# Farama-Foundation/Procgen2

Measured on AMD Instinct MI355X. Metric: env-steps/sec at 65536 envs, 64x64x3 obs, higher is better.
Workload: dtype u8/f32; 1 GPU; coinrun, 65536 envs per GPU, uniform random actions 0..14 from a device counter hash, next-step auto-reset, seeds 1+global env index; game=coinrun, distribution_mode=default, envs_per_gpu=65536, obs=64x64x3 uint8, parallelism=env-shard x1, no collective

## Files before the change

procgen2_amd/csrc/coinrun.hip:

```cpp
#include "../../include/procgen2_vec.h"
#include "pg_engine.h"
#include "pg_frame.h"
#include "pg_geom.h"
#include "pg_order.h"
#include "pg_prefetch.h"
#include "pg_prepass.h"
#include "pg_render.h"
#include "pg_rng.h"
#include "pg_tiles.h"

namespace pg {
namespace PG_VARIANT_NS {
namespace coinrun {

constexpr int W = 64, H = 64;
constexpr int kMaxEnt = 36;
constexpr int kSparks = 10;
constexpr int kSparkRow = 12;

enum Tile : uint8_t { kEmpty = 0, kWallTop, kWallMid, kLavaTop, kLavaMid, kCrate };
enum Solid { kPass = 0, kFull, kOneWay };
enum Kind { kSaw = 0, kMob = 1, kCoin = 2 };

enum Tex {
// ... 836 lines not shown
#pragma unroll
    for (int ss = 0; ss < 4; ss++) {
        bx[ss] = SC(s, SC_AX + ss, env) + -0.5f;
        by[ss] = SC(s, SC_AY + ss, env) + -1.0f;
    }
    int hazard = 0;
    if (cand0 | cand1) {
        SCI(s, SC_CAND, env) = 0;
        SCI(s, SC_CAND + 1, env) = 0;
    }
    if (bits & kBitsFar) {
        const int n_ent = SI(s, I_NENT, env);
        for (int e = 0; e < n_ent; e++) {
            float hb[6];
            entity_step<false>(s, env, e, src, 4, hb);
            hazard |= hazard_hits(hb, bx, by);
        }
    } else {
        unsigned long long cand = cand0 | (static_cast<unsigned long long>(cand1) << 32);
        while (cand) {
            const int e = __builtin_ctzll(cand);
            cand &= cand - 1;
            const float4 x = s.hazx[size_t(e) * s.n + env];
            const float2 y = s.hazy[size_t(e) * s.n + env];
            const float hb[6] = {x.x, x.y, x.z, x.w, y.x, y.y};
            hazard |= hazard_hits(hb, bx, by);
        }
    }
    const int lava = (bits >> 8) & 15, coin = (bits >> 12) & 15;
    const int ending = hazard | lava | coin;
    const int last = ending ? __builtin_ctz(ending) : 3;
    SCI(s, SC_REDO, env) = last < 3 ? last + 1 : 0;
    const bool alive = !(((hazard | lava) >> last) & 1);
    const bool got_coin = ((coin >> last) & 1) != 0;
    const float ax = SC(s, SC_AX + last, env), ay = SC(s, SC_AY + last, env);
    SF(s, F_AX, env) = ax;
    SF(s, F_AY, env) = ay;
    SF(s, F_AVX, env) = SC(s, SC_AVX + last, env);
    SF(s, F_AVY, env) = SC(s, SC_AVY + last, env);
    SF(s, F_APHASE, env) = SC(s, SC_PHASE + last, env);
    SF(s, F_CAMX, env) = ax * kUnitPx;
    SF(s, F_CAMY, env) = (ay - 0.5f) * kUnitPx;
    SI(s, I_FLAGS, env) = kFlagListed | (((bits >> last) & 1) ? kFlagGround : 0) |
                          (((bits >> (4 + last)) & 1) ? kFlagForward : 0) | (src ? 0 : kFlagBuf);
    const bool terminated = !alive || got_coin;
    io.reward[env] = got_coin * 10.0f;
    io.done[env] = terminated ? 1 : 0;
    io.pending[env] = terminated ? reset_due_mark(step_index + 1u) : 0;
}

constexpr int kRenderWaves = 2;
#ifndef PG_COINRUN_QUARTERS
#define PG_COINRUN_QUARTERS false
#endif
constexpr bool kQuarters = PG_COINRUN_QUARTERS;

#ifndef PG_COINRUN_RENDER_WAVES
#define PG_COINRUN_RENDER_WAVES 5
#endif
constexpr int kGrid = 16;

PG_D int tile_tex(int tile, int crate, int ground_theme) {
    return tile == kWallMid   ? kTexMid + ground_theme
           : tile == kWallTop ? kTexTop + ground_theme
           : tile == kLavaMid ? kTexLava
           : tile == kLavaTop ? kTexLavaTop
                              : kTexCrate + crate;
}
PG_D int kind_tex(int k, int ground_theme) { return tile_tex(k < 4 ? k + 1 : kCrate, (k - 4) & 3, ground_theme); }
PG_D DrawCall spark_draw(float life, float x, float y, const int4& d) {
    if (!(life > 0.0f)) return kNoDraw;
    const float lr = (5.0f - life) / 5.0f;
    const float alpha = 0.5f * (1.0f - lr);
    const float scale = 0.45f * (0.4f * lr + 0.6f);
    const float oy = -lr * 0.17f;
    return DrawCall{true, false, false, kTexSpark, x * kUnitPx - 0.5f * d.y * scale, (y + oy) * kUnitPx - 0.5f * d.z * scale,
                    scale * kUnitPx / d.y, alpha, 0.0f};
}
PG_D int sprite_tex(int tex0, int dyn) { return (dyn & kDynTexSet) ? tex0 + ((dyn & kDynFrame) ? 1 : 0) : 0; }
PG_D DrawCall sprite_draw(int dyn, float x, float y, int tex, const int4& d) {
    if (!(dyn & kDynTexSet)) return kNoDraw;
    const float scale = 1.0f * 1.0f;
    return DrawCall{true, (dyn & kDynFlip) != 0, false, tex, (x + -0.5f) * kUnitPx, (y + -0.5f) * kUnitPx, scale * kUnitPx / d.y, 1.0f, 0.0f};
}
PG_D int agent_tex(int sflags, float avx, float aphase, int alien) {
    const bool ground = (sflags & kFlagGround) != 0;
    if (fabsf(avx) < 0.01f && ground) return kTexStand + alien;
    if (!ground) return kTexJump + alien;
    return (aphase > 0.5f ? kTexWalk2 : kTexWalk1) + alien;
}
PG_D DrawCall agent_draw(int sflags, float ax, float ay, int tex, const int4& d) {
    const float px = ax - 0.5f, py = ay - 2.0f;
    return DrawCall{true, (sflags & kFlagForward) == 0, false, tex, px * kUnitPx, py * kUnitPx, kUnitPx / d.y, 1.0f, 0.0f};
}

PG_D void render_full(const State& s, const AtlasView& atlas, const StepIO& io, int flags, int env, uint32_t* fb,
                      ComposeLds<kGrid>& L) {
    const int lane = threadIdx.x & 63, half = __builtin_amdgcn_readfirstlane(threadIdx.x >> 6);
    constexpr int halves = kRenderWaves;
    uint32_t* const slots = fb + kFbWords - kBlitWords * 64;
    static_assert(sizeof(ComposeTmp<kGrid>) + sizeof(ComposeHand) + kBlitWords * 64 * 4 <= kFbWords * 4, "room behind the set-up tables");

    const Camera cam{SF(s, F_CAMX, env), SF(s, F_CAMY, env), 64.0f, 64.0f, 0.3f * 64.0f / 64.0f};
    const int themes = SI(s, I_THEMES, env);
    const int sflags = SI(s, I_FLAGS, env);
    const int buf = (sflags & kFlagBuf) ? 1 : 0;
    const int backdrop = PG_ABL(flags, 16) ? 9 : (themes & 0xff);
    const int alien = (themes >> 8) & 0xff, ground_theme = (themes >> 16) & 0xff;
    const int n_ent = SI(s, I_NENT, env);
    const int n_mob = SI(s, I_NMOB, env);
    const uint8_t* tiles = s.tiles + size_t(env) * (W * H);
    const DescRegs descs = DescRegs::load(atlas, lane);
    Blit mine;
    PG_MARK("a_state");

    {
        const int redo = SCI(s, SC_REDO, env);
        __syncthreads();
        if (redo) {
            if (half == 0 && lane < n_ent) {
                float hb[6];
                entity_step(s, env, lane, 1 - buf, redo, hb);
            }
            if (threadIdx.x == 0) SCI(s, SC_REDO, env) = 0;
            __threadfence();
            __syncthreads();
        }
    }

    const int n_parts = n_mob * kSparks;
    const int n_sprites = (sflags & kFlagListed) ? n_ent : 0;
    const bool one_pass = n_parts + n_sprites + 1 <= 64;
    const int first_sprite = one_pass ? n_parts : 0;
    const bool is_part = one_pass && lane < n_parts;
    const bool is_sprite = lane >= first_sprite && lane < first_sprite + n_sprites;
    const bool is_agent = lane == first_sprite + n_sprites;
    int spr_e = 0, spr_dyn = 0, spr_tex = 0;
    float spr_x = 0.0f, spr_y = 0.0f, part_life = 0.0f, part_x = 0.0f, part_y = 0.0f;
    if (half != 1) {
    } else if (is_sprite) {
        spr_e = EB(s, EB_DRAW_ORDER, lane - first_sprite, env);
        spr_dyn = DB(s, buf, spr_e, env);
        spr_tex = EB(s, EB_TEX, spr_e, env);
        spr_x = DF(s, buf, DF_X, spr_e, env);
        spr_y = EY(s, spr_e, env);
    } else if (is_part) {
        const int m = lane / kSparks, k = lane - m * kSparks;
        const int e = EB(s, EB_SPARK_ORDER, m, env);
        part_life = SP(s, buf, 2, e, k, env);
        part_x = SP(s, buf, 0, e, k, env);
        part_y = SP(s, buf, 1, e, k, env);
    }
    PG_MARK("b_inputs");

    const BgDraw bg_draw = backdrop_draw(descs.uniform(kTexBackdrop + backdrop), SF(s, F_BGSHIFT, env));
    const int4& bg_d = bg_draw.desc;

    const TileWindow win = tile_window(cam);
    const int x0 = win.x0, y0 = win.y0;
    const int cols = win.x1 - x0 + 1, rows = win.y1 - y0 + 1, cells = cols * rows;
    const int4 tile_desc = descs.uniform(kTexMid);

    if (half == 1 && !PG_ABL(flags, 2)) {
        {
            bool has = false;
            int want_tex = 0;
            if (is_part)
                want_tex = kTexSpark;
            else if (is_sprite)
                want_tex = sprite_tex(spr_tex, spr_dyn);
            else if (is_agent)
                want_tex = agent_tex(sflags, SF(s, F_AVX, env), SF(s, F_APHASE, env), alien);
            const int4 d = descs.at(want_tex);
            DrawCall c = kNoDraw;
            if (is_part)
                c = spark_draw(part_life, part_x, part_y, d);
            else if (is_sprite)
                c = sprite_draw(spr_dyn, spr_x, spr_y, want_tex, d);
            else if (is_agent)
                c = agent_draw(sflags, SF(s, F_AX, env), SF(s, F_AY, env), want_tex, d);
            if (c.go) has = resolve_draw(cam, d.y, d.z, d.x, c.wx, c.wy, c.scale, c.alpha, c.flip_h, false, mine);
            blit_share(slots, lane, mine, has);
        }
    }
    PG_MARK("c_resolve");
    BgAxis bga{};
    bool composed = false, sprites_ready = false;
    ReplayState<4> sprite_pass;
    if (!(flags & 1) && !PG_ABL(flags, 4) && cols <= kGrid && rows <= kGrid) {
        compose_spans(fb, L, cam, x0, y0, cols, rows, tile_desc.y, tile_desc.z, kUnitPx / tile_desc.y, lane, 0, half, halves,
                      0, 0, &bg_draw, &bga);
    PG_MARK("d_spans");
        const int4 kind_d = descs.at(kind_tex(lane & 7, ground_theme));
        const int kind_base = kind_d.x;
        uint32_t soft_rows = (threadIdx.x == 0 && bg_d.w != 0) ? 0x80000000u : 0u;
        const uint32_t hard_rows = (threadIdx.x == 0 && (bg_d.w & 2)) ? 0x80000000u : 0u;
#pragma unroll
        for (int k = 0; k < kGrid * kGrid / 64; k++) {
            if (half != 0) break;
            const int cell = k * 64 + lane;
            const int r = cell / kGrid, c = cell % kGrid;
            const int x = x0 + c, ty = H - 1 - (y0 + r);
            int raw = kWallMid;
            if (x >= 0 && ty >= 0 && x < W && ty < H) raw = tiles[ty + x * H];
            const int t = raw & 7;
            const int slot = t < kCrate ? t - 1 : 4 + (raw >> 4);
            const int off = __shfl(kind_base, slot < 0 ? 0 : slot);
            const int soft = __shfl(kind_d.w, slot < 0 ? 0 : slot);
            L.base[cell] = (t == kEmpty) ? static_cast<int32_t>(kNoTexel) : off * 4;
            if (t != kEmpty && soft != 0 && r < rows && c < cols) soft_rows |= 1u << r;
        }
        if (soft_rows) atomicOr(&L.soft_rows[half], static_cast<int32_t>(soft_rows));
        if (hard_rows) atomicOr(&L.hard_rows[half], static_cast<int32_t>(hard_rows));
        __syncthreads();
        PG_MARK("e_cells");
        sprites_ready = !PG_ABL(flags, 2);
        if (sprites_ready) {
            const bool has = blit_take(slots, lane, mine);
            sprite_pass = replay_begin(atlas, mine, __ballot(has), lane, half * (kObsH / halves), (half + 1) * (kObsH / halves));
        }
        PG_MARK("f_begin");
        composed = compose_rows(fb, L, atlas, bga, cols, rows, tile_desc.y, lane, flags, half, halves);
        PG_MARK("k_composed");
    }
    if (PG_ABL(flags, 4)) composed = true;
    bool taken = false;
    if (!composed) {
        if (!sprites_ready) {
            __syncthreads();
            taken = blit_take(slots, lane, mine);
            __syncthreads();
        }
        Blit tile;
        wave_clear(fb, lane, half, halves);
        const bool has_bg = resolve_draw(cam, bg_d.y, bg_d.z, bg_d.x, bg_draw.px, bg_draw.py, bg_draw.scale, 1.0f, false, false, tile);
        wave_replay(fb, atlas, tile, has_bg ? 1ull : 0ull, lane, half, halves);
        for (int base = 0; base < cells; base += 64) {
            const int cell = base + lane;
            bool has = false;
            if (cell < cells) {
                const int row = cell / cols;
                const int x = x0 + (cell - row * cols), y = y0 + row;
                const int ty = H - 1 - y;
                int t = kWallMid, crate = 0;
                if (x >= 0 && ty >= 0 && x < W && ty < H) {
                    const int raw = tiles[ty + x * H];
                    t = raw & 7;
                    crate = raw >> 4;
                }
                if (t != kEmpty) {
                    const int4 d = atlas.desc[tile_tex(t, crate, ground_theme)];
                    has = resolve_draw(cam, d.y, d.z, d.x, x * kUnitPx, y * kUnitPx, kUnitPx / d.y, 1.0f, false, false,
                                       tile);
                }
            }
            wave_replay(fb, atlas, tile, __ballot(has), lane, half, halves);
        }
    }

    if (!PG_ABL(flags, 2)) {
        const int4 spark_d = descs.uniform(kTexSpark);
        if (!one_pass) {
            Blit spark;
            for (int base = 0; base < n_parts; base += 64) {
                bool has = false;
                if (base + lane < n_parts) {
                    const int idx = base + lane, m = idx / kSparks, k = idx - m * kSparks;
                    const int e = EB(s, EB_SPARK_ORDER, m, env);
                    const DrawCall c = spark_draw(SP(s, buf, 2, e, k, env), SP(s, buf, 0, e, k, env), SP(s, buf, 1, e, k, env), spark_d);
                    has = c.go && resolve_draw(cam, spark_d.y, spark_d.z, spark_d.x, c.wx, c.wy, c.scale, c.alpha, false, false, spark);
                }
                wave_replay_rows(fb, atlas, spark, __ballot(has), lane, half * (kObsH / halves), (half + 1) * (kObsH / halves));
            }
        }
        if (!sprites_ready)
            sprite_pass = replay_begin(atlas, mine, __ballot(taken), lane, half * (kObsH / halves), (half + 1) * (kObsH / halves));
        PG_MARK("m_fallback_and_rounds");
        replay_finish(fb, atlas, mine, sprite_pass, lane, half * (kObsH / halves), (half + 1) * (kObsH / halves));
        PG_MARK("n_sprites");
    }
    if (!PG_ABL(flags, 8))
        wave_store_rows(fb, io.obs + size_t(env) * kObsBytes, lane, half * (kObsH / halves), (half + 1) * (kObsH / halves));
    PG_MARK("o_store");
}

constexpr int kPrepEnvs = 8, kPrepThreads = 256;
constexpr int kSlotTop = 0, kSlotMid = 1, kSlotLavaTop = 2, kSlotLava = 3, kSlotCrate = 4;

struct PrepEnv {
    int32_t sflags, buf, n_ent, n_mob, n_sprites, alien;
    float avx, aphase, ax, ay;
};
struct SetupLds {
    PrepLds<kGrid, kPrepEnvs, kMaxSpan> P;
    PrepEnv env[kPrepEnvs];
    int4 desc[kTexCount];
    uint8_t order[kPrepEnvs][2][kMaxEnt + 4];
    int32_t kind_soft[kPrepEnvs];
    uint32_t row_valid[kPrepEnvs][kGrid / 4];
    int32_t counts[kPrepEnvs];
    PrepDrawQueue queue[kPrepThreads / 64];
};

__global__ void __launch_bounds__(kPrepThreads) setup_kernel(State s, AtlasView atlas, const uint8_t* mask, int flags) {
    __shared__ SetupLds S;
    PrepLds<kGrid, kPrepEnvs, kMaxSpan>& P = S.P;
    const int tid = threadIdx.x, lane = tid & 63, wave = __builtin_amdgcn_readfirstlane(tid >> 6);
    const int env0 = prep_block(blockIdx.x, gridDim.x) * kPrepEnvs;
    const PrepOut& out = s.prep;

    for (int q = tid; q < kPrepEnvs * 2 * 64; q += kPrepThreads) (&P.cover[0][0][0])[q] = 0u;
    if (tid < kTexCount) S.desc[tid] = atlas.desc[tid];
    static_assert(kTexCount <= kPrepThreads, "one descriptor per thread");
    for (int q = tid; q < kPrepEnvs * 2 * kMaxEnt; q += kPrepThreads) {
        const int e = q / (2 * kMaxEnt), r = q - e * (2 * kMaxEnt), which = r / kMaxEnt, j = r - which * kMaxEnt;
        if (env0 + e < s.n) S.order[e][which][j] = EB(s, which ? EB_DRAW_ORDER : EB_SPARK_ORDER, j, env0 + e);
    }
    Camera cam{};
    int themes = 0, redo = 0;
    float bgshift = 0.0f;
    bool active = false;
    if (tid < kPrepEnvs) {
        const int e = tid, env = env0 + e;
        active = env < s.n && (!mask || mask[env]);
        if (active) {
            redo = SCI(s, SC_REDO, env);
            cam = Camera{SF(s, F_CAMX, env), SF(s, F_CAMY, env), 64.0f, 64.0f, 0.3f * 64.0f / 64.0f};
            themes = SI(s, I_THEMES, env);
            bgshift = SF(s, F_BGSHIFT, env);
            PrepEnv pe{};
            pe.sflags = SI(s, I_FLAGS, env);
            pe.buf = (pe.sflags & kFlagBuf) ? 1 : 0;
            pe.n_ent = SI(s, I_NENT, env);
            pe.n_mob = SI(s, I_NMOB, env);
            pe.n_sprites = (pe.sflags & kFlagListed) ? pe.n_ent : 0;
            pe.alien = (themes >> 8) & 0xff;
            pe.avx = SF(s, F_AVX, env);
            pe.aphase = SF(s, F_APHASE, env);
            pe.ax = SF(s, F_AX, env);
            pe.ay = SF(s, F_AY, env);
            S.env[e] = pe;
        }
    }
    __syncthreads();
    if (tid < kPrepEnvs) {
        const int e = tid;
        PrepView v{};
        P.fat[e] = 0;
        P.soft_rows[e] = P.hard_rows[e] = 0;
        S.counts[e] = 0;
        S.kind_soft[e] = 0;
        if (active && redo != 0) {
            P.fat[e] = 1;
            active = false;
        }
        if (active) {
            v.cam = cam;
            const int4 d = S.desc[kTexBackdrop + (PG_ABL(flags, 16) ? 9 : (themes & 0xff))];
            v.bg = backdrop_draw(d, bgshift);
            const TileWindow win = tile_window(cam);
            v.x0 = win.x0;
            v.y0 = win.y0;
            v.cols = win.x1 - win.x0 + 1;
            v.rows = win.y1 - win.y0 + 1;
            const int4 tile_desc = S.desc[kTexMid];
            v.tw = tile_desc.y;
            v.th = tile_desc.z;
            v.th2 = 0;
            v.tile_scale = kUnitPx / tile_desc.y;
            if (v.cols > kGrid || v.rows > kGrid || ((flags & kDebugFatThirds) && (env0 + e) % 3 == 0)) {
                P.fat[e] = 1;
                active = false;
            }
            P.soft_rows[e] = d.w != 0 ? 0x80000000u : 0u;
            P.hard_rows[e] = (d.w & 2) ? 0x80000000u : 0u;
            const int ground_theme = (themes >> 16) & 0xff;
            int soft = 0;
#pragma unroll
            for (int k = 0; k < 8; k++) {
                const int4 kd = S.desc[kind_tex(k, ground_theme)];
                P.meta[e][PM_KINDS + k] = static_cast<uint32_t>(kd.x) * 4u;
                    if (kd.w != 0) soft |= 1 << k;
            }
            S.kind_soft[e] = soft;
            prep_row_valid<kGrid, H>(v.y0, S.row_valid[e]);
        }
        v.active = active ? 1 : 0;
        P.view[e] = v;
    }
    __syncthreads();
    if (PG_ABL(flags, 0x1000000)) return;

    static_assert(kGrid == 16 && H == 64, "a window column is one 16-byte load");
    const int cell_e = tid / kGrid, cell_c = tid - cell_e * kGrid;
    bool cell_lane = false, cell_x_ok = false;
    uint32_t column[kGrid / 4] = {};
    if (tid < kPrepEnvs * kGrid && P.view[cell_e].active) {
        cell_lane = true;
        prep_column_fetch<kGrid, W, H>(s.tiles + size_t(env0 + cell_e) * (W * H), P.view[cell_e].x0 + cell_c, P.view[cell_e].y0, cell_x_ok, column);
    }
    if (!PG_ABL(flags, 0x2000000)) prep_spans<kGrid, kMaxSpan, kPrepEnvs>(P, tid, kPrepThreads);
    if (cell_lane) {
        const PrepView& v = P.view[cell_e];
        uint32_t in_rows[4];
        prep_column_rows<kGrid>(column, S.row_valid[cell_e], cell_x_ok, kWallMid, in_rows);
        const uint32_t soft_kinds = static_cast<uint32_t>(S.kind_soft[cell_e]);
        uint32_t soft_lo = 0u, soft_hi = 0u;
#pragma unroll
        for (int k = 0; k < 4; k++) {
            soft_lo |= ((soft_kinds >> k) & 1u) ? 0xffu << (8 * k) : 0u;
            soft_hi |= ((soft_kinds >> (4 + k)) & 1u) ? 0xffu << (8 * k) : 0u;
        }
        uint32_t kinds[4], soft_rows = 0u;
#pragma unroll
        for (int w = 0; w < 4; w++) {
            const uint32_t raw = in_rows[w];
            const uint32_t t = raw & 0x07070707u, crate = (raw >> 4) & 0x03030303u;
            const uint32_t y = (t | 0x80808080u) - 0x01010101u;
            const uint32_t there = ((y & 0x80808080u) >> 7) * 0xffu;
            const uint32_t slots = (y & 0x07070707u) + crate;
            kinds[w] = (slots & there) | ~there;
            const uint32_t sel = (slots & there) | (0x0c0c0c0cu & ~there);
            const uint32_t soft = __builtin_amdgcn_perm(soft_hi, soft_lo, sel) & 0x01010101u;
            soft_rows |= ((soft * 0x00204081u >> 21) & 0xfu) << (4 * w);
        }
        if (cell_c >= v.cols) soft_rows = 0u;
        soft_rows &= (v.rows >= 32 ? ~0u : (1u << v.rows) - 1u);
        prep_column_store<kGrid>(out.cells + size_t(env0 + cell_e) * (kGrid * kGrid), cell_c, kinds);
        if (soft_rows) atomicOr(&P.soft_rows[cell_e], soft_rows);
    }
    __syncthreads();
    if (PG_ABL(flags, 0x4000000)) return;
    if (!PG_ABL(flags, 0x8000000)) prep_axes<kGrid, kMaxSpan, kPrepEnvs>(P, out, env0, wave, kPrepThreads / 64, lane);
    if (PG_ABL(flags, 0x10000000)) return;

    static_assert(kPrepEnvs == 2 * (kPrepThreads / 64), "two envs per wavefront");
    {
        const int ea = 2 * wave, eb = 2 * wave + 1;
        const bool on_a = P.view[ea].active != 0, on_b = P.view[eb].active != 0;
        const Camera cam_a = P.view[ea].cam, cam_b = P.view[eb].cam;
        const int cnt_a = on_a ? S.env[ea].n_mob * kSparks + S.env[ea].n_sprites + 1 : 0;
        const int cnt_b = on_b ? S.env[eb].n_mob * kSparks + S.env[eb].n_sprites + 1 : 0;
        uint32_t* const draws_a = out.draws + size_t(env0 + ea) * kPrepDraws * kBlitWords;
        uint32_t* const draws_b = out.draws + size_t(env0 + eb) * kPrepDraws * kBlitWords;
        PrepDrawPass st{0, {0, 0}, {0, 0}};
        PrepDrawQueue& Q = S.queue[wave];
        for (int base = 0; base < cnt_a + cnt_b; base += 64) {
            const int q = base + lane;
            const bool is_b = q >= cnt_a;
            const int e = is_b ? eb : ea, env = env0 + e;
            const int slot = is_b ? q - cnt_a : q;
            const bool valid = q < cnt_a + cnt_b;
            const PrepEnv& pe = S.env[e];
            const int n_parts = pe.n_mob * kSparks;
            DrawCall p = kNoDraw;
            if (valid && slot < n_parts) {
                const int m = slot / kSparks, k = slot - m * kSparks;
                const int ent = S.order[e][0][m];
                const float life = SP(s, pe.buf, 2, ent, k, env);
                const float px = SP(s, pe.buf, 0, ent, k, env), py = SP(s, pe.buf, 1, ent, k, env);
                p = spark_draw(life, px, py, S.desc[kTexSpark]);
            } else if (valid && slot < n_parts + pe.n_sprites) {
                const int ent = S.order[e][1][slot - n_parts];
                const int dyn = DB(s, pe.buf, ent, env);
                const int tex0 = EB(s, EB_TEX, ent, env);
                const float ex = DF(s, pe.buf, DF_X, ent, env), ey = EY(s, ent, env);
                const int tex = sprite_tex(tex0, dyn);
                p = sprite_draw(dyn, ex, ey, tex, S.desc[tex]);
            } else if (valid) {
                const int tex = agent_tex(pe.sflags, pe.avx, pe.aphase, pe.alien);
                p = agent_draw(pe.sflags, pe.ax, pe.ay, tex, S.desc[tex]);
            }
            prep_draws_pass(Q, st, S.desc, cam_a, cam_b, draws_a, draws_b, valid, is_b, p, lane);
        }
        prep_draws_flush(Q, st, S.desc, cam_a, cam_b, draws_a, draws_b, lane);
        if (lane == 0) {
            S.counts[ea] = st.done[0];
            S.counts[eb] = st.done[1];
        }
    }
    __syncthreads();
    prep_meta_out<kGrid, kMaxSpan, kPrepEnvs>(P, out, env0, S.counts, tid, kPrepThreads);
}

__global__ void __launch_bounds__(64 * kRenderWaves, PG_COINRUN_RENDER_WAVES) render_kernel(State s, AtlasView atlas, const uint8_t* mask,
                                                                   StepIO io, int flags) {
    const int env = blockIdx.x;
    if (mask && !mask[env]) return;
    const int lane = threadIdx.x & 63, half = __builtin_amdgcn_readfirstlane(threadIdx.x >> 6);
    constexpr int halves = kRenderWaves;
    __shared__ alignas(16) uint32_t fb[kFbWords];
    __shared__ ComposeLds<kGrid> L;
    PG_TL_BEGIN(6);
    PG_TL(0);
    const PrepMeta M{s.prep.meta + size_t(env) * kPrepMetaWords};
    const uint32_t colw = s.prep.axes[size_t(env) * 128 + lane], roww = s.prep.axes[size_t(env) * 128 + 64 + lane];
    const uint32_t kind_off = M.w[PM_KINDS + (lane & (kPrepKinds - 1))];
    const uint32_t two = reinterpret_cast<const uint16_t*>(s.prep.cells)[size_t(env) * (kGrid * kGrid / 2) + half * 64 + lane];
    const int n_draws = M.draws();
    const bool has = lane < n_draws;
    const Blit mine = prep_draw_load(s.prep.draws + (size_t(env) * kPrepDraws + lane) * kBlitWords, has);
    prep_cells_expand<kGrid>(L, two, kind_off, half, lane);
    const ComposeRegs R = prep_regs<kGrid>(M, colw, roww, 0u, lane);
    __syncthreads();
    PG_TL(1);
    if ((flags & (1 | kDebugNoPrepass)) || M.fat()) {
        render_full(s, atlas, io, flags, env, fb, L);
        return;
    }
    const int row_lo = half * (kObsH / halves), row_hi = (half + 1) * (kObsH / halves);
    ReplayState<4> sprite_pass = replay_begin<4, false, true, false, kQuarters>(atlas, mine, PG_ABL(flags, 2) ? 0ull : __ballot(has), lane, row_lo, row_hi);
    PG_TL(2);
    if (!PG_ABL(flags, 4)) compose_rows_from<kGrid, false, false>(fb, L, atlas, R, lane, flags, half, halves);
    PG_TL(3);
    replay_finish<4, false, true, 4, false, kQuarters>(fb, atlas, mine, sprite_pass, lane, row_lo, row_hi);
    PG_TL(4);
    if (!PG_ABL(flags, 8)) wave_store_rows(fb, io.obs + size_t(env) * kObsBytes, lane, row_lo, row_hi);
    PG_TL_END(6, true, io.obs + size_t(env) * kObsBytes + half * (kObsBytes / 2));
}

template <class Painter>
__device__ void frame_draws(const State& s, const AtlasView& atlas, int env, Painter& P) {
    const float fw = P.width(), fh = P.height();
    P.begin(atlas, Camera{SF(s, F_CAMX, env), SF(s, F_CAMY, env), fw, fh, 0.3f * fw / 64.0f});
    const int themes = SI(s, I_THEMES, env), sflags = SI(s, I_FLAGS, env);
    const int buf = (sflags & kFlagBuf) ? 1 : 0;
    const int backdrop = themes & 0xff, alien = (themes >> 8) & 0xff, ground_theme = (themes >> 16) & 0xff;
    const uint8_t* tiles = s.tiles + size_t(env) * (W * H);
    P.clear();
    const BgDraw bg = backdrop_draw(P.desc(kTexBackdrop + backdrop), SF(s, F_BGSHIFT, env));
    P.draw(kTexBackdrop + backdrop, bg.px, bg.py, bg.scale);
    const TileWindow win = P.window();
    for (int y = win.y0; y <= win.y1; y++)
        for (int x = win.x0; x <= win.x1; x++) {
            const int ty = H - 1 - y;
            int t_id = kWallMid, crate = 0;
            if (x >= 0 && ty >= 0 && x < W && ty < H) {
                const int raw = tiles[ty + x * H];
                t_id = raw & 7;
                crate = raw >> 4;
            }
            if (t_id == kEmpty) continue;
            const int tex = tile_tex(t_id, crate, ground_theme);
            P.draw(tex, x * kUnitPx, y * kUnitPx, kUnitPx / P.desc(tex).y);
        }
    const int n_mob = SI(s, I_NMOB, env);
    for (int m = 0; m < n_mob; m++) {
        const int e = EB(s, EB_SPARK_ORDER, m, env);
        for (int k = 0; k < kSparks; k++)
            P.draw(spark_draw(SP(s, buf, 2, e, k, env), SP(s, buf, 0, e, k, env), SP(s, buf, 1, e, k, env), P.desc(kTexSpark)));
    }
    const int n_sprites = (sflags & kFlagListed) ? SI(s, I_NENT, env) : 0;
    for (int k = 0; k < n_sprites; k++) {
        const int e = EB(s, EB_DRAW_ORDER, k, env);
        const int dyn = DB(s, buf, e, env);
        const int tex = sprite_tex(EB(s, EB_TEX, e, env), dyn);
        P.draw(sprite_draw(dyn, DF(s, buf, DF_X, e, env), EY(s, e, env), tex, P.desc(tex)));
    }
    const int tex = agent_tex(sflags, SF(s, F_AVX, env), SF(s, F_APHASE, env), alien);
    P.draw(agent_draw(sflags, SF(s, F_AX, env), SF(s, F_AY, env), tex, P.desc(tex)));
}

__global__ void __launch_bounds__(kFrameThreads) frame_kernel(State s, AtlasView atlas, int env, FrameTarget t) {
    FramePainter P(t);
    frame_draws(s, atlas, env, P);
}

__global__ void __launch_bounds__(kFrameThreads) frames_kernel(State s, AtlasView atlas, FrameBatch fb) {
    __shared__ uint32_t tile[kTilePx];
    TilePainter P(tile, fb);
    const int env = P.env(fb);
    if (env >= 0) frame_draws(s, atlas, env, P);
    P.store(fb);
}

class CoinrunGame final : public PrefetchingGame<Gen> {
   public:
    const char* name() const override { return "coinrun"; }
    bool set_game_flags(uint32_t flags) override {
        const uint32_t known = PGV_COINRUN_NO_PIT | PGV_COINRUN_NO_CRATE | PGV_COINRUN_NO_DY | PGV_COINRUN_NO_MOBS;
        s_.no = flags & known;
        return (flags & ~known) == 0;
    }

    std::vector<std::string> texture_names() const override {
        static const char* themes[6] = {"Dirt", "Grass", "Planet", "Sand", "Snow", "Stone"};
        static const char* walkers[9] = {"slimeBlock", "slimePurple", "slimeBlue", "slimeGreen", "mouse",
                                         "snail",      "ladybug",     "wormGreen", "wormPink"};
        static const char* crates[4] = {"boxCrate", "boxCrate_double", "boxCrate_single", "boxCrate_warning"};
        static const char* aliens[5] = {"Beige", "Blue", "Green", "Pink", "Yellow"};
        std::vector<std::string> v;
        auto lower = [](std::string t) {
            for (auto& ch : t) ch = static_cast<char>(tolower(ch));
            return t;
        };
        for (auto t : themes) v.push_back(std::string("kenney/Ground/") + t + "/" + lower(t) + "Mid.png");
        for (auto t : themes) v.push_back(std::string("kenney/Ground/") + t + "/" + lower(t) + "Center.png");
        v.push_back("kenney/Tiles/lavaTop_low.png");
        v.push_back("kenney/Tiles/lava.png");
        for (auto c : crates) v.push_back(std::string("kenney/Tiles/") + c + ".png");
        for (auto w : walkers) {
            v.push_back(std::string("kenney/Enemies/") + w + ".png");
            v.push_back(std::string("kenney/Enemies/") + w + "_move.png");
        }
        v.push_back("kenney/Enemies/sawHalf.png");
        v.push_back("kenney/Enemies/sawHalf_move.png");
        v.push_back("kenney/Items/coinGold.png");
        for (auto pose : {"_stand.png", "_jump.png", "_walk1.png", "_walk2.png"})
            for (auto a : aliens) v.push_back(std::string("kenney/Players/128x256/") + a + "/alien" + a + pose);
        v.push_back("misc_assets/iconCircle_white.png");
        for (const char* b : {"alien_bg", "another_world_bg", "back_cave", "caverns", "cyberpunk_bg", "parallax_forest",
                              "scifi_bg", "scifi2_bg", "living_tissue_bg", "airadventurelevel1", "airadventurelevel2",
                              "airadventurelevel3", "airadventurelevel4", "cave_background", "blue_desert",
                              "blue_grass", "blue_land", "blue_shroom", "colored_desert", "colored_grass",
                              "colored_land", "colored_shroom", "landscape1", "landscape2", "landscape3",
                              "landscape4", "battleback1", "battleback2", "battleback3", "battleback4", "battleback5",
                              "battleback6", "battleback7", "battleback8", "battleback9", "battleback10", "sunrise"})
            v.push_back(std::string("platform_backgrounds/") + b + ".png");
        for (const char* fam : {"beach", "fantasy", "candy"})
            for (int k = 1; k <= 4; k++)
                v.push_back(std::string("platform_backgrounds_2/") + fam + std::to_string(k) + ".png");
        return v;
    }

    std::string check_atlas(const std::vector<std::pair<int, int>>& sizes) const override {
        if (static_cast<int>(sizes.size()) != kTexCount) return "coinrun: unexpected texture count";
        for (int t = kTexTop; t < kTexWalker; t++)
            if (sizes[t] != sizes[kTexMid]) return "coinrun: tile textures differ in size";
        return "";
    }

    static void carve(Carve& c, State& s, int n) {
        c.take_env(s.shadow, n, 1, sizeof(Level));
        c.take_env(s.slot, n, 1, 4);
        c.take_env(s.mt, n, 1, kMtWords * 4);
        c.take_env(s.tiles, n, 1, W * H);
        c.take_env(s.f, n, F_COUNT, 4);
        c.take_env(s.i, n, I_COUNT, 4);
        c.take_env(s.ey, n, kMaxEnt, 4);
        c.take_env(s.eb, n, EB_COUNT * kMaxEnt, 1);
        c.take_env(s.df, n, 2 * DF_COUNT * kMaxEnt, 4);
        c.take_env(s.db, n, 2 * kMaxEnt, 1);
        c.take_env(s.spark, n, 2, 3 * kMaxEnt * kSparkRow * 4);
        c.take_env(s.scratch, n, SC_COUNT, 4);
    }
    size_t state_bytes(int n) const override { return Carve::size(carve, n); }
    void bind(void* d_state, int n, AtlasView atlas) override {
        Carve::bind(carve, d_state, s_, n, &regions);
        s_.n = n;
        atlas_ = atlas;
    }
    int blocks() const { return (s_.n + 63) / 64; }
    void launch_make(hipStream_t st, uint32_t seed_base, int env_offset) override {
        hipLaunchKernelGGL(make_kernel, dim3(blocks()), dim3(64), 0, st, s_, seed_base, env_offset);
        make_levels(st, seed_base, env_offset);
    }
    void launch_logic(hipStream_t st, const int32_t* actions, uint32_t run_seed, uint32_t step_index, int env_offset,
                      StepIO io) override {
        const bool fused = prefetch() != 0;
        reset_before_logic(st, step_index, io);
        const dim3 blocks((s_.n + 63) / 64, 2 + kMobRows + kStaticRows);
        const float reach_x = (debug_flags & kDebugCoinrunNoReach) ? 0.0f : kReachX;
        const float reach_y = (debug_flags & kDebugCoinrunNoReach) ? 0.0f : kReachY;
        hipLaunchKernelGGL(logic_kernel, blocks, dim3(64), 0, st, s_, actions, run_seed, step_index, env_offset, io,
                           prefetch(), plan, fused ? 1 : 0, reach_x, reach_y);
        hipLaunchKernelGGL(resolve_kernel, dim3((s_.n + 63) / 64, fused ? 2 : 1), dim3(64), 0, st, s_, io, step_index, prefetch(),
                           plan);
    }
    bool launch_frame(hipStream_t st, int env, uint32_t* d_px, int w, int h) override {
        hipLaunchKernelGGL(frame_kernel, dim3(1), dim3(kFrameThreads), 0, st, s_, atlas_, env, FrameTarget{d_px, w, h});
        return true;
    }
    void launch_frames(hipStream_t st, const int32_t* d_indices, int count, uint8_t* d_rgb, int w, int h) override {
        launch_frames_tiled(frames_kernel, st, s_, atlas_, d_indices, count, d_rgb, w, h, s_.n);
    }
    void launch_prepass(hipStream_t st, const uint8_t* mask) override {
        if (!(debug_flags & (1 | kDebugNoPrepass)) && !PG_ABL(debug_flags, 1 << 22))
            hipLaunchKernelGGL(setup_kernel, dim3((s_.n + kPrepEnvs - 1) / kPrepEnvs), dim3(kPrepThreads), 0, st, s_, atlas_, mask, debug_flags);
    }
    void launch_render(hipStream_t st, const uint8_t* mask, StepIO io) override {
        hipLaunchKernelGGL(render_kernel, dim3(s_.n), dim3(64 * kRenderWaves), 0, st, s_, atlas_, mask, io,
                           debug_flags);
    }
    static void carve_scratch(Carve& c, State& s, int n) {
        prep_carve(c, s.prep, n, kGrid, kBlitWords, false);
        c.take(s.hazx, size_t(kMaxEnt) * n * sizeof(float4));
        c.take(s.hazy, size_t(kMaxEnt) * n * sizeof(float2));
    }
    size_t scratch_bytes(int n) const override { return Carve::size(carve_scratch, n); }
    void bind_scratch(void* d_scratch, int n) override { Carve::bind(carve_scratch, d_scratch, s_, n); }

    int dump_state(hipStream_t st, int env, float* out, int cap) override {
        hipStreamSynchronize(st);
        const size_t n = s_.n;
        auto f = [&](int field) { return read_one(s_.f + size_t(field) * n + env); };
        auto ri = [&](int field) { return read_one(s_.i + size_t(field) * n + env); };
        const int flags = ri(I_FLAGS), themes = ri(I_THEMES), n_ent = ri(I_NENT);
        const int buf = (flags & kFlagBuf) ? 1 : 0;
        std::vector<float> v = {f(F_AX), f(F_AY), f(F_AVX), f(F_AVY), (flags & kFlagGround) ? 1.0f : 0.0f,
                                (flags & kFlagForward) ? 1.0f : 0.0f, f(F_APHASE), f(F_CAMX), f(F_CAMY),
                                static_cast<float>(themes & 0xff), f(F_BGSHIFT), static_cast<float>((themes >> 8) & 0xff),
                                static_cast<float>((themes >> 16) & 0xff), static_cast<float>(n_ent)};
        for (int e = 0; e < n_ent; e++) {
            const int kind = read_one(s_.eb + (size_t(EB_KIND) * kMaxEnt + e) * n + env);
            const int dyn = read_one(s_.db + (size_t(buf) * kMaxEnt + e) * n + env);
            auto df = [&](int field) { return read_one(s_.df + ((size_t(buf) * DF_COUNT + field) * kMaxEnt + e) * n + env); };
            v.push_back(df(DF_X));
            v.push_back(read_one(s_.ey + size_t(e) * n + env));
            v.push_back(kind == kMob ? df(DF_VX) : 0.0f);
            v.push_back((dyn & kDynFrame) ? 1.0f : 0.0f);
            v.push_back(kind == kCoin ? 0.0f : df(DF_ANIM_T));
        }
        return dump_out(v, out, cap);
    }
    int dump_tiles(hipStream_t st, int env, uint8_t* out, int cap) override {
        return dump_env_tiles(st, s_.tiles, W * H, W * H, env, out, cap, 7);
    }

   private:
    AtlasView atlas_{};
};

}

}

std::unique_ptr<Game> PG_FACTORY(make_coinrun)() { return std::make_unique<PG_VARIANT_NS::coinrun::CoinrunGame>(); }

}
```

Measured before the change: 141.9 million env-steps/s.

## Run deferred entity substeps in setup kernel and split full-render path into own kernel

Envs with pending redo substeps now have their entity stepping finished inside the setup prepass, so they can follow the fast prepass render path instead of being marked fat. The heavy render_full fallback moves into a separate render_full_kernel used only when prepass is disabled, and fat envs in render_kernel use a lighter painter-based draw. This shrinks the register and LDS footprint of the main render kernel. setup_kernel also gets a min-blocks launch bound of 8, which may cap its registers. The cost is extra divergent work and a global write with a fence in setup.

```diff
diff --git a/procgen2_amd/csrc/coinrun.hip b/procgen2_amd/csrc/coinrun.hip
--- a/procgen2_amd/csrc/coinrun.hip
+++ b/procgen2_amd/csrc/coinrun.hip
@@ -1162,7 +1162,7 @@
     PrepDrawQueue queue[kPrepThreads / 64];
 };
 
-__global__ void __launch_bounds__(kPrepThreads) setup_kernel(State s, AtlasView atlas, const uint8_t* mask, int flags) {
+__global__ void __launch_bounds__(kPrepThreads, 8) setup_kernel(State s, AtlasView atlas, const uint8_t* mask, int flags) {
     __shared__ SetupLds S;
     PrepLds<kGrid, kPrepEnvs, kMaxSpan>& P = S.P;
     const int tid = threadIdx.x, lane = tid & 63, wave = __builtin_amdgcn_readfirstlane(tid >> 6);
@@ -1202,7 +1202,38 @@
             S.env[e] = pe;
         }
     }
+    if (wave == 0) {
+        const bool owed = __ballot(redo != 0) != 0;
+        if (lane == 0) S.order[0][0][kMaxEnt] = owed ? 1 : 0;
+    }
     __syncthreads();
+    if (__builtin_amdgcn_readfirstlane(S.order[0][0][kMaxEnt])) {
+        if (wave == 0) {
+            uint32_t owed = 0u;
+#pragma unroll
+            for (int e = 0; e < kPrepEnvs; e++) owed |= static_cast<uint32_t>(__builtin_amdgcn_readlane(redo, e)) << (4 * e);
+            if (redo != 0) SCI(s, SC_REDO, env0 + tid) = 0;
+#pragma unroll 1
+            for (int e = 0; e < kPrepEnvs; e++) {
+                const int n_sub = (owed >> (4 * e)) & 15;
+                if (n_sub != 0 && lane < S.env[e].n_ent) {
+                    float hb[6];
+                    entity_step(s, env0 + e, lane, 1 - S.env[e].buf, n_sub, hb);
+                }
+            }
+        }
+        __threadfence();
+        __syncthreads();
+        if (tid < kPrepEnvs) {
+            const int env = env0 + tid;
+            active = env < s.n && (!mask || mask[env]);
+            if (active) {
+                cam = Camera{SF(s, F_CAMX, env), SF(s, F_CAMY, env), 64.0f, 64.0f, 0.3f * 64.0f / 64.0f};
+                themes = SI(s, I_THEMES, env);
+                bgshift = SF(s, F_BGSHIFT, env);
+            }
+        }
+    }
     if (tid < kPrepEnvs) {
         const int e = tid;
         PrepView v{};
@@ -1210,10 +1241,6 @@
         P.soft_rows[e] = P.hard_rows[e] = 0;
         S.counts[e] = 0;
         S.kind_soft[e] = 0;
-        if (active && redo != 0) {
-            P.fat[e] = 1;
-            active = false;
-        }
         if (active) {
             v.cam = cam;
             const int4 d = S.desc[kTexBackdrop + (PG_ABL(flags, 16) ? 9 : (themes & 0xff))];
@@ -1343,6 +1370,28 @@
     prep_meta_out<kGrid, kMaxSpan, kPrepEnvs>(P, out, env0, S.counts, tid, kPrepThreads);
 }
 
+template <class Painter>
+__device__ void frame_draws(const State& s, const AtlasView& atlas, int env, Painter& P);
+
+struct ObsPainter : PainterCalls<ObsPainter> {
+    uint32_t* fb;
+    int tid;
+    PG_D explicit ObsPainter(uint32_t* target) : fb(target), tid(static_cast<int>(threadIdx.x)) {}
+    PG_D float width() const { return static_cast<float>(kObsW); }
+    PG_D float height() const { return static_cast<float>(kObsH); }
+    PG_D bool lead() const { return tid == 0; }
+    PG_D void clear() {
+        for (int k = tid; k < kFbWords; k += 64 * kRenderWaves) fb[k] = 0u;
+        __syncthreads();
+    }
+    PG_D void blit(const Blit& b) {
+        PixRect r = draw_reach(b);
+        if (!rect_clip(r, PixRect{0, 0, kObsW - 1, kObsH - 1})) return;
+        paint_rect(b, atlas.texels, r, fb, kObsW, 0, 0, tid, 64 * kRenderWaves);
+        __syncthreads();
+    }
+};
+
 __global__ void __launch_bounds__(64 * kRenderWaves, PG_COINRUN_RENDER_WAVES) render_kernel(State s, AtlasView atlas, const uint8_t* mask,
                                                                    StepIO io, int flags) {
     const int env = blockIdx.x;
@@ -1364,8 +1413,11 @@
     const ComposeRegs R = prep_regs<kGrid>(M, colw, roww, 0u, lane);
     __syncthreads();
     PG_TL(1);
-    if ((flags & (1 | kDebugNoPrepass)) || M.fat()) {
-        render_full(s, atlas, io, flags, env, fb, L);
+    if (M.fat()) {
+        __syncthreads();
+        ObsPainter P(fb);
+        frame_draws(s, atlas, env, P);
+        wave_store_rows(fb, io.obs + size_t(env) * kObsBytes, lane, half * (kObsH / halves), (half + 1) * (kObsH / halves));
         return;
     }
     const int row_lo = half * (kObsH / halves), row_hi = (half + 1) * (kObsH / halves);
@@ -1377,6 +1429,15 @@
     PG_TL(4);
     if (!PG_ABL(flags, 8)) wave_store_rows(fb, io.obs + size_t(env) * kObsBytes, lane, row_lo, row_hi);
     PG_TL_END(6, true, io.obs + size_t(env) * kObsBytes + half * (kObsBytes / 2));
+}
+
+__global__ void __launch_bounds__(64 * kRenderWaves, PG_COINRUN_RENDER_WAVES) render_full_kernel(State s, AtlasView atlas, const uint8_t* mask,
+                                                                        StepIO io, int flags) {
+    const int env = blockIdx.x;
+    if (mask && !mask[env]) return;
+    __shared__ alignas(16) uint32_t fb[kFbWords];
+    __shared__ ComposeLds<kGrid> L;
+    render_full(s, atlas, io, flags, env, fb, L);
 }
 
 template <class Painter>
@@ -1534,13 +1595,18 @@
     void launch_frames(hipStream_t st, const int32_t* d_indices, int count, uint8_t* d_rgb, int w, int h) override {
         launch_frames_tiled(frames_kernel, st, s_, atlas_, d_indices, count, d_rgb, w, h, s_.n);
     }
+    bool lean() const { return !(debug_flags & (1 | kDebugNoPrepass)); }
     void launch_prepass(hipStream_t st, const uint8_t* mask) override {
-        if (!(debug_flags & (1 | kDebugNoPrepass)) && !PG_ABL(debug_flags, 1 << 22))
+        if (lean() && !PG_ABL(debug_flags, 1 << 22))
             hipLaunchKernelGGL(setup_kernel, dim3((s_.n + kPrepEnvs - 1) / kPrepEnvs), dim3(kPrepThreads), 0, st, s_, atlas_, mask, debug_flags);
     }
     void launch_render(hipStream_t st, const uint8_t* mask, StepIO io) override {
-        hipLaunchKernelGGL(render_kernel, dim3(s_.n), dim3(64 * kRenderWaves), 0, st, s_, atlas_, mask, io,
-                           debug_flags);
+        if (lean())
+            hipLaunchKernelGGL(render_kernel, dim3(s_.n), dim3(64 * kRenderWaves), 0, st, s_, atlas_, mask, io,
+                               debug_flags);
+        else
+            hipLaunchKernelGGL(render_full_kernel, dim3(s_.n), dim3(64 * kRenderWaves), 0, st, s_, atlas_, mask, io,
+                               debug_flags);
     }
     static void carve_scratch(Carve& c, State& s, int n) {
         prep_carve(c, s.prep, n, kGrid, kBlitWords, false);
```

Result: slower. 89.69 million env-steps/s (-36.8%).
